# brodbeck-m/dolfinx_eqlb

Measured on AMD Instinct MI355X. Metric: equilibrated patches/s (fp64) on 1M-tri Poisson k=2; L2 flux-divergence residual, higher is better.
Workload: dtype f64; 1 GPU; Poisson 1000000 triangles per GPU (crossed unit square 500x500), P2 primal, FluxEqlbSE RT2, homogeneous Dirichlet, fp64; headline=True, patches_per_gpu=501001, cells_per_gpu=1000000, nrhs=1, weak_symmetry=False, partition=none, solver=shuffle, scatter=tiled, accumulate=True

## Files before the change

### dolfinx_eqlb_amd/csrc/eqlb_internal.h

```cpp
#pragma once

#include <hip/hip_runtime.h>

#include <cstdint>
#include <string>
#include <map>
#include <mutex>
#include <vector>

#include "../../include/eqlb.h"

namespace eqlb
{

constexpr uint32_t INFO_FM_SHIFT = 0, INFO_FP_SHIFT = 2, INFO_LN_SHIFT = 4;
constexpr uint32_t INFO_REV_M = 1u << 6, INFO_REV_P = 1u << 7;
constexpr uint32_t INFO_LOCAL_SHIFT = 8;

constexpr uint8_t PFLAG_INTERIOR = 1, PFLAG_BC0 = 2, PFLAG_BCN = 4;
constexpr uint8_t PFLAG_WS_SKIP = 8, PFLAG_WS_GROUP = 16;
constexpr uint8_t PFLAG_WS_LEVEL_SHIFT = 5;
constexpr int WS_MAX_LEVELS = 4;
constexpr uint32_t INFO_GROUPROW_SHIFT = 8;

// ... 73 lines not shown
#endif
__host__ __device__ constexpr bool tile_spec_full(int K, int P) { return P <= 8 && K >= 2; }
__host__ __device__ constexpr bool tile_spec_interior(int K, int P)
{
  return EQLB_TILE_INTERIOR && ((K == 2 && (P == 8 || P == 16)) || (EQLB_TILE_INTERIOR_K3 && K == 3 && P == 8));
}
__host__ __device__ __forceinline__ int tile_wb_all(int n, int P) { return (n * P + 63) >> 6; }
__host__ __device__ __forceinline__ int tile_wb_whole(int n, int P) { return (n * P) >> 6; }
template <int P>
__host__ __device__ __forceinline__ void tile_nfix_range(const TileDesc& td, int B, int j, int& c0, int& c1)
{
  constexpr int PER = 64 / P;
  const int first = (j == 0) ? td.nfull[B] : td.nval[B][j - 1];
  c0 = (first + PER - 1) / PER;
  c1 = (EQLB_STRESS_NFIX && P - 1 - j >= 3) ? td.nval[B][j] / PER : 0;
  if (c1 < c0)
    c1 = c0;
}

struct TileArgs
{
  const TileDesc* tiles;
  const int32_t* tile_cells;
  int32_t ntiles, tc;
  const int32_t* facet_owner;
  const int32_t* cell_dofs;
  int64_t ndofs;
  int32_t nfacets;
  int32_t tile_first;
  int32_t accumulate;
  const double* basis_C;
  const double* basis_R;
};

constexpr int MULTI_RHS_MAX = 8;
struct MultiRhs
{
  int32_t n, rhs0;
  const double* g[MULTI_RHS_MAX];
  const double* f[MULTI_RHS_MAX];
  double* x[MULTI_RHS_MAX];
};

struct BuildArgs
{
  int32_t nnodes, nfacets, nrhs;
  const int32_t *cell_nodes, *cell_facets, *facet_nodes, *facet_cells_off, *facet_cells;
  const int32_t *node_cells_off, *node_facets_off, *node_facets;
  const uint8_t* facet_perm;
  const int8_t* facet_type;
  const int64_t* node_slot;
  const int64_t* node_patch;
  int64_t npatch_total;
  int32_t* slot_cell;
  uint32_t* slot_info;
  uint8_t* pn;
  uint8_t* pflag;
  const int8_t* node_ws;
  const int32_t* node_group;
  const int8_t* node_wslevel;
  int64_t ninst;
  const int32_t* inst_node;
  const int32_t* inst_slot;
  const int32_t* inst_tile;
  const int32_t* cell_tile;
  const int32_t* cell_pos;
  int32_t tile_cells;
  int32_t stride;
  int32_t *ex_ncells, *ex_cells, *ex_fcts;
  int8_t *ex_fl, *ex_il, *ex_rev;
  int32_t large;
};

void launch_build_patches(const BuildArgs& a, hipStream_t stream);
void launch_cell_geometry(int32_t ncells, const double* x, const int32_t* cell_nodes,
                          double* cellJ, hipStream_t stream);
int launch_se_patch(int k, int deg, int P, int solver, int scatter, const SeArgs& a,
                    hipStream_t stream, int mode = 0);
int launch_se_patch_fused(int k, int deg, int scatter, const SeArgs& a, const FusedBins& fb,
                          hipStream_t stream);
int launch_se_patch_tiled(int k, int deg, int mode, const SeArgs& a, const TileArgs& t, hipStream_t stream);
int launch_se_patch_tiled_multi(int k, int deg, int mode, const SeArgs& a, const TileArgs& t, const MultiRhs& mr,
                                hipStream_t stream);
int launch_se_patch_lowdeg(int k, int deg, int P, int solver, int scatter, const SeArgs& a, hipStream_t stream,
                           int mode);
int launch_se_patch_fused_lowdeg(int k, int deg, int scatter, const SeArgs& a, const FusedBins& fb,
                                 hipStream_t stream);
int launch_se_patch_tiled_lowdeg(int k, int deg, int mode, const SeArgs& a, const TileArgs& t, hipStream_t stream);
int launch_se_patch_tiled_multi_lowdeg(int k, int deg, int mode, const SeArgs& a, const TileArgs& t,
                                       const MultiRhs& mr, hipStream_t stream);
int launch_ev_patch_fused_lowdeg(int k, int deg, const SeArgs& a, const FusedBins& fb, hipStream_t stream);
int launch_se_patch_k4_lowdeg(int deg, int P, int solver, int scatter, const SeArgs& a, hipStream_t stream,
                              int mode);
int fill_tables_k4_lowdeg(int deg, std::vector<double>& out);
void launch_tile_facet_owner(const DeviceMesh& m, int64_t n, const int32_t* tile_cells, int32_t* code,
                             hipStream_t stream);
int tile_cells_of(int k);
int tile_cells_ev_of(int k);
int tile_cells_max_of(int k);
int launch_se_patch_large(int k, int deg, int mode, const SeArgs& a, const int32_t* off, double* ws,
                          hipStream_t stream);
size_t large_patch_ws_doubles(int k, int64_t nslots, int64_t npatch);
int launch_se_weaksym_large(int k, const SeArgs& a, const int32_t* off, const int64_t* wsoff, double* ws,
                            hipStream_t stream);
size_t large_patch_weaksym_ws_doubles(int k, int64_t ncells_of_patch);
int launch_se_weaksym(int k, int P, bool no_flux_bcs, const SeArgs& a, hipStream_t stream);
int launch_se_weaksym_banded(int k, int P, const SeArgs& a, hipStream_t stream);
int launch_se_stress_tiled(const SeArgs& a, const TileArgs& t, const double* const* g, const double* const* f,
                           double* const* x, hipStream_t stream, bool mixed = false);
int stress_tile_cells();
int launch_ev_patch_fused(int k, int deg, const SeArgs& a, const FusedBins& fb, hipStream_t stream);
void launch_ev_boundary_to_broken(const DeviceMesh& m, int k, int nrhs, const int32_t* cell_dofs,
                                  int64_t ndofs, const double* bv_conf, double* bv_broken,
                                  const double* facet_maps, hipStream_t stream);
void launch_ev_reduce(const DeviceMesh& m, int k, int nrhs, const int32_t* cell_dofs, int64_t ndofs,
                      const double* slots, double* x, int accumulate, const double* basis_C, const double* basis_R,
                      hipStream_t stream);
int launch_reduce_slots(int nrt, int32_t ncells, int32_t nrhs, const double* slots, double* x, int accumulate,
                        hipStream_t stream);
int launch_reduce_slots_cells(int nrt, int32_t ncells, int64_t nlist, const int32_t* cells, const double* slots,
                              double* x, hipStream_t stream);
int projection_matrix_host(int degree, int nq, const double* pts, const double* wts,
                           std::vector<double>& Pm);
void launch_project_dg(int64_t ncells, int nd, int nq, int bs, const double* Pm, const double* qv,
                       double* out, hipStream_t stream);
void launch_korn(const DeviceMesh& m, const int64_t* node_slot, const int64_t* node_patch,
                 const int32_t* slot_cell, const uint32_t* slot_info, const uint8_t* pn,
                 const uint8_t* pflag, double* cks, double* korn, hipStream_t stream, int64_t l_npatch = 0,
                 const int32_t* l_nodes = nullptr, const int32_t* l_off = nullptr, const int32_t* l_slot_cell = nullptr,
                 const uint32_t* l_slot_info = nullptr, const uint8_t* l_pflag = nullptr);
int launch_estimate(const DeviceMesh& m, int k, int deg, int nrhs, const double* x_eq, const double* flux_dg,
                    const double* rhs_dg, double* div2, double* sig2, double* jump, double alpha,
                    double beta, hipStream_t stream);
int launch_boundary_residual(const DeviceMesh& m, int k, int deg, int nrhs, const double* x_eq,
                             const double* flux_dg, int32_t nlist, const int32_t* facets, const double* bvals,
                             double* out, hipStream_t stream);
int launch_estimate_stress(const DeviceMesh& m, const int32_t* node_cells, int k, const double* x0,
                           const double* x1, const double* korn, double pi_1, double* energy, double* wsym,
                           double* node_asym, hipStream_t stream);
int launch_oscillation(const DeviceMesh& m, int k, int deg, int nrhs, const double* x_eq, const double* flux_dg,
                       int nq, const double* qpoints, const double* qweights, const double* fvalues,
                       const double* korn, double* out, hipStream_t stream);
int launch_estimate_lowdeg(const DeviceMesh& m, int k, int deg, int nrhs, const double* x_eq, const double* flux_dg,
                           const double* rhs_dg, double* div2, double* sig2, double* jump, double alpha,
                           double beta, hipStream_t stream);
int launch_boundary_residual_lowdeg(const DeviceMesh& m, int k, int deg, int nrhs, const double* x_eq,
                                    const double* flux_dg, int32_t nlist, const int32_t* facets,
                                    const double* bvals, double* out, hipStream_t stream);
int launch_oscillation_lowdeg(const DeviceMesh& m, int k, int deg, int nrhs, const double* x_eq,
                              const double* flux_dg, int nq, const double* qpoints, const double* qweights,
                              const double* fvalues, const double* korn, double* out, hipStream_t stream);
int launch_estimate_k4_lowdeg(const DeviceMesh& m, int deg, int nrhs, const double* x_eq, const double* flux_dg,
                              const double* rhs_dg, double* div2, double* sig2, double* jump, double alpha,
                              double beta, hipStream_t stream);
int launch_boundary_residual_k4_lowdeg(const DeviceMesh& m, int deg, int nrhs, const double* x_eq,
                                       const double* flux_dg, int32_t nlist, const int32_t* facets,
                                       const double* bvals, double* out, hipStream_t stream);
int launch_oscillation_k4_lowdeg(const DeviceMesh& m, int deg, int nrhs, const double* x_eq, const double* flux_dg,
                                 int nq, const double* qpoints, const double* qweights, const double* fvalues,
                                 const double* korn, double* out, hipStream_t stream);
int set_error(int code, const char* fmt, ...);
void launch_halo_pack(int nrhs, int32_t nlist, int32_t nrt, int64_t ncells, const int64_t* cells, double* x,
                      double* buf, int clear, hipStream_t stream);
void launch_halo_unpack_add(int nrhs, int32_t nlist, int32_t nrt, int64_t ncells, const int64_t* cells,
                            double* x, const double* buf, hipStream_t stream);
void device_tiling_prepare();
// ... 115 lines not shown
```

### dolfinx_eqlb_amd/csrc/eqlb_se_kernels.hip

```cpp
#include "eqlb_device_common.h"
#include "eqlb_tables_gen.h"

#ifndef EQLB_PCR_SELECTS
#define EQLB_PCR_SELECTS 0
#endif

#ifndef EQLB_SE_TEMPLATES_ONLY
#define EQLB_SE_TEMPLATES_ONLY 0
#endif

namespace eqlb
{

#if !EQLB_SE_TEMPLATES_ONLY
size_t table_doubles(int k, int deg)
{
  const int nrt = nrt_of(k), nd = nd_of(deg), nq = nq_of(k);
  const int kb = k - 1, nadd = (k - 1) * (k - 2) / 2, ndiv = k * (k + 1) / 2 - 1;
  const int nh = 1 + 2 * kb + nadd, ncol = 2 * k + ndiv;
  const int hrow = nd * nq + ((nd * nq) & 1);
  const int nte = nh * (nh + 1) / 2;
  return (size_t)3 * nrt * nrt + (size_t)9 * nd * k + (size_t)3 * hrow + (size_t)6 * nd * nq
         + (size_t)NCOMBO * 3 * (nte + (nte & 1)) + (size_t)NCOMBO * 3 * nh * (ncol + (ncol & 1))
         + (size_t)9 * k * k + (size_t)3 * nrt * 2 + (size_t)NCOMBO * 2 * nh * 3
// ... 1841 lines not shown
{
  const int64_t e = (int64_t)blockIdx.x * blockDim.x + threadIdx.x;
  if (e >= n)
    return;
  const int32_t c = tile_cells[e / 3];
  const int lf = (int)(e % 3);
  int32_t v = -1;
  if (c >= 0)
  {
    const int32_t fct = cell_facets[(int64_t)c * 3 + lf];
    if (facet_cells[facet_cells_off[fct]] == c)
      v = 2 * fct + (facet_perm[(int64_t)c * 3 + lf] ? 1 : 0);
  }
  code[e] = v;
}

void launch_tile_facet_owner(const DeviceMesh& m, int64_t n, const int32_t* tile_cells, int32_t* code,
                             hipStream_t stream)
{
  if (n > 0)
    hipLaunchKernelGGL(k_tile_facet_owner, dim3((unsigned)((n + 255) / 256)), dim3(256), 0, stream, n,
                       tile_cells, m.cell_facets, m.facet_cells_off, m.facet_cells, m.facet_perm, code);
}
#endif

__device__ __forceinline__ int xcd_remap(int b, int n)
{
#if EQLB_XCD_REMAP
  const int q = n / 8, r = n % 8, x = b % 8;
  return ((x < r) ? x * (q + 1) : r * (q + 1) + (x - r) * q) + b / 8;
#else
  return b;
#endif
}

template <int K, int NPK>
__device__ __forceinline__ double packed_sum(const double* rows, int i)
{
  if (i >= 3 * K)
  {
    const int q = i - K;
    return (rows[q] + rows[NPK + q]) + rows[2 * NPK + q];
  }
  const int f = i / K, j = i - f * K;
  const int la = (f == 0) ? 1 : 0, lb = (f == 2) ? 1 : 2;
  return rows[la * NPK + (f - ((f > la) ? 1 : 0)) * K + j] + rows[lb * NPK + (f - ((f > lb) ? 1 : 0)) * K + j];
}

template <int K, int DEG, int MODE>
__device__ __forceinline__ void tile_stage(const SeArgs& a0, const TileArgs& ta, const int tile, double* lds)
{
  constexpr int TILE_THREADS = tile_threads_c(K);
  using Z = Sizes<K, DEG, 8>;
  constexpr int NRT = Z::NRT;
  const int TC = ta.tc;
  constexpr int NPK = NRT - K;
  constexpr bool HALFWQ = K == 3;
  constexpr int NTABL = HALFWQ ? Z::NTAB_HALF : Z::NTAB;
  constexpr int NTABM = NTABL + (MODE ? Z::NEV : 0);
  double* sSlots = lds + NTABM;
  if constexpr (HALFWQ)
  {
    constexpr int NHEAD = Z::NF + Z::NHT + Z::NDT + Z::NTET;
    constexpr int NCMB = Z::NCMB;
    for (int i = threadIdx.x; i < NHEAD; i += TILE_THREADS)
      lds[i] = a0.tables[Z::NS + i];
    for (int i = threadIdx.x; i < (NCOMBO / 2) * NCMB; i += TILE_THREADS)
      lds[NHEAD + (i / NCMB) * Z::NCMBH + (i % NCMB)] = a0.tables[Z::NS + NHEAD + (i / NCMB) * 2 * NCMB + (i % NCMB)];
    for (int i = threadIdx.x; i < Z::NHB; i += TILE_THREADS)
      lds[NHEAD + Z::NWQH + i] = a0.tables[Z::NS + NHEAD + Z::NWQT + i];
  }
  else
    for (int i = threadIdx.x; i < Z::NTAB; i += TILE_THREADS)
      lds[i] = a0.tables[Z::NS + i];
  if constexpr (MODE == 1)
    for (int i = threadIdx.x; i < Z::NEV; i += TILE_THREADS)
      lds[NTABL + i] = a0.tables[Z::OFF_HG + i];
  if (ta.tiles[tile].zero)
    for (int i = threadIdx.x; i < TC * 3 * NPK; i += TILE_THREADS)
      sSlots[i] = 0.0;
  __syncthreads();
}

template <int K, int DEG, int MODE>
__device__ __forceinline__ void tile_sweep_flush(const SeArgs& a0, const TileArgs& ta, const int tile, double* lds)
{
  constexpr int TILE_THREADS = tile_threads_c(K);
  using Z = Sizes<K, DEG, 8>;
  constexpr int NRT = Z::NRT;
  constexpr int TCMAX = tile_cells_max_c(K);
  const int TC = ta.tc;
  constexpr int NPK = NRT - K;
  constexpr bool HALFWQ = K == 3;
  constexpr int NTABL = HALFWQ ? Z::NTAB_HALF : Z::NTAB;
  constexpr int NTABM = NTABL + (MODE ? Z::NEV : 0);
  double* sSlots = lds + NTABM;
  const TileDesc& td = ta.tiles[tile];
#ifndef EQLB_TILE_SOLVER
#define EQLB_TILE_SOLVER 1
#endif
#ifndef EQLB_EXP_FULLONLY
#define EQLB_EXP_FULLONLY 0
#endif
  const int wave = threadIdx.x >> 6, lane = threadIdx.x & 63;
  constexpr int NW = TILE_THREADS / 64;
  int u = wave;
  SeArgs a = a0;
#define EQLB_TILE_BIN(B, PP)                                                                        \
  {                                                                                                 \
    const int np = td.npatch[B];                                                                    \
    const int nwb = tile_wb_all(np, PP);                                                            \
    a.npatch = np;                                                                                  \
    a.slot_offset = td.slot_start[B];                                                               \
    a.patch_offset = td.patch_start[B];                                                             \
     \
    constexpr bool SPEC = tile_spec_full(K, PP);                                                    \
    const int nwb_full = SPEC ? tile_wb_whole(td.nfull[B], PP) : 0;                                 \
     \
    constexpr bool SPECI = tile_spec_interior(K, PP);                                               \
    const int nwb_int = SPECI ? tile_wb_whole(td.nint[B], PP) : 0;                                  \
    for (; u < nwb; u += NW)                                                                        \
    {                                                                                               \
      if (u < nwb_full)                                                                             \
        se_patch_body<K, DEG, PP, EQLB_TILE_SOLVER, 2, 64, MODE, SPEC>(a, 0, lds, true, (int64_t)u * 64 + lane, sSlots); \
      else if (SPECI && u < nwb_int)                                                                \
        se_patch_body<K, DEG, PP, EQLB_TILE_SOLVER, 2, 64, MODE, false, SPECI>(a, 0, lds, true, (int64_t)u * 64 + lane, sSlots); \
      else if (!EQLB_EXP_FULLONLY)             \
        se_patch_body<K, DEG, PP, EQLB_TILE_SOLVER, 2, 64, MODE>(a, 0, lds, true, (int64_t)u * 64 + lane, sSlots); \
    }                                                                                               \
    u -= nwb;                                                                                       \
  }
#ifndef EQLB_EXP_NOBODY
  EQLB_TILE_BIN(0, 4)
  EQLB_TILE_BIN(1, 8)
  EQLB_TILE_BIN(2, 16)
  EQLB_TILE_BIN(3, 32)
  EQLB_TILE_BIN(4, 64)
#else
  (void)u;
  (void)lane;
  (void)td;
#endif
#undef EQLB_TILE_BIN
  const int32_t* cells = ta.tile_cells + (int64_t)tile * TC;
  const bool conforming = MODE == 1 && ta.facet_owner != nullptr;
  double* x = a0.out + (int64_t)a0.rhs_out * a0.ncells * NRT;
  constexpr int VW = (NRT % 2 == 0) ? 2 : 1;
  constexpr int NIT = (TCMAX * NRT / VW + TILE_THREADS - 1) / TILE_THREADS;
  double xv[NIT][VW];
  int64_t xi[NIT];
  if (!conforming)
  {
#pragma unroll
    for (int it = 0; it < NIT; ++it)
    {
      const int e = (it * TILE_THREADS + threadIdx.x) * VW;
      const int cl = e / NRT, i = e - cl * NRT;
      const int32_t cell = (e < TC * NRT) ? cells[cl] : -1;
      xi[it] = (cell >= 0) ? (int64_t)cell * NRT + i : -1;
    }
#pragma unroll
    for (int it = 0; it < NIT; ++it)
    {
#ifdef EQLB_EXP_NOXREAD
      xv[it][0] = xv[it][VW - 1] = 0.0;
      continue;
#endif
      if (!ta.accumulate)
      {
        xv[it][0] = xv[it][VW - 1] = 0.0;
        continue;
      }
      if constexpr (VW == 2)
      {
#if EQLB_FLUSH_NT
        xv[it][0] = (xi[it] >= 0) ? __builtin_nontemporal_load(x + xi[it]) : 0.0;
        xv[it][1] = (xi[it] >= 0) ? __builtin_nontemporal_load(x + xi[it] + 1) : 0.0;
#else
        const double2 t = (xi[it] >= 0) ? *reinterpret_cast<const double2*>(x + xi[it]) : make_double2(0.0, 0.0);
        xv[it][0] = t.x;
        xv[it][1] = t.y;
#endif
      }
      else
        xv[it][0] = (xi[it] >= 0) ? x[xi[it]] : 0.0;
    }
  }
  constexpr int NIC = K * K - K;
  constexpr int NFE = (TCMAX * 3 + TILE_THREADS - 1) / TILE_THREADS;
  constexpr int NIE = (NIC > 0) ? (TCMAX * NIC + TILE_THREADS - 1) / TILE_THREADS : 1;
  int32_t fcode[NFE];
  int64_t fdof[NFE];
  double fold[NFE][K];
  int64_t idof[NIE];
  double iold[NIE];
  const bool conf_plain = conforming && ta.basis_C == nullptr;
  if (conf_plain)
  {
    const double* xc0 = a0.out + (int64_t)a0.rhs_out * ta.ndofs;
    const int32_t* own0 = ta.facet_owner + (int64_t)tile * TC * 3;
#pragma unroll
    for (int it = 0; it < NFE; ++it)
    {
      const int e = it * TILE_THREADS + threadIdx.x;
      fcode[it] = (e < TC * 3) ? own0[e] : -1;
    }
#pragma unroll
    for (int it = 0; it < NFE; ++it)
    {
      const int e = it * TILE_THREADS + threadIdx.x;
      const int cl = e / 3, lf = e - 3 * cl;
      fdof[it] = -1;
      if (fcode[it] >= 0)
        fdof[it] = ta.cell_dofs ? (int64_t)cells[cl] * NRT + lf * K : (int64_t)(fcode[it] >> 1) * K;
#pragma unroll
      for (int j = 0; j < K; ++j)
      {
        fold[it][j] = 0.0;
        if (fcode[it] >= 0 && ta.accumulate)
          fold[it][j] = ta.cell_dofs ? xc0[ta.cell_dofs[fdof[it] + j]] : xc0[fdof[it] + j];
      }
    }
    if constexpr (NIC > 0)
    {
#pragma unroll
      for (int it = 0; it < NIE; ++it)
// ... 184 lines not shown
  using Z = Sizes<K, DEG, 8>;
  const size_t lds_bytes
      = sizeof(double) * ((size_t)(K == 3 ? Z::NTAB_HALF : Z::NTAB) + (MODE ? (size_t)Z::NEV : 0) + (size_t)t.tc * 3 * (Z::NRT - K));
  if (lds_bytes > 160 * 1024 || t.tc < 1 || t.tc > tile_cells_max_c(K) || mr.n < 1 || mr.n > MULTI_RHS_MAX)
    return EQLB_ERR_UNSUPPORTED;
  auto kern = k_se_patch_tiled_multi<K, DEG, MODE>;
  if (lds_bytes > 64 * 1024)
  {
    if (hipFuncSetAttribute(reinterpret_cast<const void*>(kern),
                            hipFuncAttributeMaxDynamicSharedMemorySize, (int)lds_bytes) != hipSuccess)
      return EQLB_ERR_DEVICE;
  }
  if (t.ntiles == 0)
    return 0;
  hipLaunchKernelGGL(kern, dim3((unsigned)t.ntiles * (unsigned)mr.n), dim3(tile_threads_c(K)), lds_bytes, stream, a, t, mr);
  return (hipGetLastError() == hipSuccess) ? 0 : EQLB_ERR_DEVICE;
}

#if !EQLB_SE_TEMPLATES_ONLY
int launch_se_patch_tiled_multi(int k, int deg, int mode, const SeArgs& a, const TileArgs& t, const MultiRhs& mr,
                                hipStream_t stream)
{
  if (deg != k - 1)
    return launch_se_patch_tiled_multi_lowdeg(k, deg, mode, a, t, mr, stream);
  if (mode == 1)
  {
    if (k == 1)
      return launch_tiled_multi_kd<1, 0, 1>(a, t, mr, stream);
    if (k == 2)
      return launch_tiled_multi_kd<2, 1, 1>(a, t, mr, stream);
    if (k == 3)
      return launch_tiled_multi_kd<3, 2, 1>(a, t, mr, stream);
    return EQLB_ERR_UNSUPPORTED;
  }
  if (k == 1 && deg == 0)
    return launch_tiled_multi_kd<1, 0, 0>(a, t, mr, stream);
  if (k == 2 && deg == 1)
    return launch_tiled_multi_kd<2, 1, 0>(a, t, mr, stream);
  if (k == 3 && deg == 2)
    return launch_tiled_multi_kd<3, 2, 0>(a, t, mr, stream);
  return EQLB_ERR_UNSUPPORTED;
}
#endif

template <int K, int DEG, int MODE>
static int launch_tiled_kd(const SeArgs& a, const TileArgs& t, hipStream_t stream)
{
  using Z = Sizes<K, DEG, 8>;
  const size_t lds_bytes
      = sizeof(double) * ((size_t)(K == 3 ? Z::NTAB_HALF : Z::NTAB) + (MODE ? (size_t)Z::NEV : 0) + (size_t)t.tc * 3 * (Z::NRT - K));
  if (lds_bytes > 160 * 1024 || t.tc < 1 || t.tc > tile_cells_max_c(K))
    return EQLB_ERR_UNSUPPORTED;
  auto kern = k_se_patch_tiled<K, DEG, MODE>;
  if (lds_bytes > 64 * 1024)
  {
    if (hipFuncSetAttribute(reinterpret_cast<const void*>(kern),
                            hipFuncAttributeMaxDynamicSharedMemorySize, (int)lds_bytes) != hipSuccess)
      return EQLB_ERR_DEVICE;
  }
  if (t.ntiles == 0)
    return 0;
  hipLaunchKernelGGL(kern, dim3((unsigned)t.ntiles), dim3(tile_threads_c(K)), lds_bytes, stream, a, t);
  return (hipGetLastError() == hipSuccess) ? 0 : EQLB_ERR_DEVICE;
}

#if !EQLB_SE_TEMPLATES_ONLY
int launch_se_patch_tiled(int k, int deg, int mode, const SeArgs& a, const TileArgs& t, hipStream_t stream)
{
  if (deg != k - 1)
    return launch_se_patch_tiled_lowdeg(k, deg, mode, a, t, stream);
  if (mode == 1)
  {
    if (k == 1)
      return launch_tiled_kd<1, 0, 1>(a, t, stream);
    if (k == 2)
      return launch_tiled_kd<2, 1, 1>(a, t, stream);
    if (k == 3)
      return launch_tiled_kd<3, 2, 1>(a, t, stream);
    return EQLB_ERR_UNSUPPORTED;
  }
  if (k == 1 && deg == 0)
    return launch_tiled_kd<1, 0, 0>(a, t, stream);
  if (k == 2 && deg == 1)
    return launch_tiled_kd<2, 1, 0>(a, t, stream);
  if (k == 3 && deg == 2)
    return launch_tiled_kd<3, 2, 0>(a, t, stream);
  return EQLB_ERR_UNSUPPORTED;
}

template <int NRT>
__global__ void __launch_bounds__(256)
k_reduce_slots(int64_t ntotal, const double* __restrict__ slots, double* __restrict__ x, int accumulate)
{
  const int64_t e = (int64_t)blockIdx.x * blockDim.x + threadIdx.x;
  if (e >= ntotal)
    return;
  const int64_t c = e / NRT;
  const int i = (int)(e - c * NRT);
  const double* s = slots + c * 3 * NRT + i;
  const double v = (s[0] + s[NRT]) + s[2 * NRT];
  x[e] = accumulate ? x[e] + v : v;
}

int launch_reduce_slots(int nrt, int32_t ncells, int32_t nrhs, const double* slots, double* x, int accumulate,
                        hipStream_t stream)
{
  const int64_t ntotal = (int64_t)nrhs * ncells * nrt;
  const int block = 256;
  const int64_t grid = (ntotal + block - 1) / block;
  if (nrt == 3)
    hipLaunchKernelGGL(k_reduce_slots<3>, dim3(grid), dim3(block), 0, stream, ntotal, slots, x, accumulate);
  else if (nrt == 8)
    hipLaunchKernelGGL(k_reduce_slots<8>, dim3(grid), dim3(block), 0, stream, ntotal, slots, x, accumulate);
  else if (nrt == 15)
    hipLaunchKernelGGL(k_reduce_slots<15>, dim3(grid), dim3(block), 0, stream, ntotal, slots, x, accumulate);
  else if (nrt == 24)
    hipLaunchKernelGGL(k_reduce_slots<24>, dim3(grid), dim3(block), 0, stream, ntotal, slots, x, accumulate);
  else
    return EQLB_ERR_UNSUPPORTED;
  return 0;
}

template <int NRT>
__global__ void __launch_bounds__(256)
k_reduce_slots_cells(int64_t ntotal, const int32_t* __restrict__ cells, const double* __restrict__ slots,
                     double* __restrict__ x)
{
  const int64_t e = (int64_t)blockIdx.x * blockDim.x + threadIdx.x;
  if (e >= ntotal)
    return;
  const int64_t c = cells[e / NRT];
  const int i = (int)(e % NRT);
  const double* s = slots + c * 3 * NRT + i;
  x[c * NRT + i] += (s[0] + s[NRT]) + s[2 * NRT];
}

int launch_reduce_slots_cells(int nrt, int32_t ncells, int64_t nlist, const int32_t* cells, const double* slots,
                              double* x, hipStream_t stream)
{
  (void)ncells;
  const int64_t ntotal = nlist * nrt;
  if (ntotal == 0)
    return 0;
  const int block = 256;
  const int64_t grid = (ntotal + block - 1) / block;
  if (nrt == 8)
    hipLaunchKernelGGL(k_reduce_slots_cells<8>, dim3(grid), dim3(block), 0, stream, ntotal, cells, slots, x);
  else if (nrt == 3)
    hipLaunchKernelGGL(k_reduce_slots_cells<3>, dim3(grid), dim3(block), 0, stream, ntotal, cells, slots, x);
  else if (nrt == 15)
    hipLaunchKernelGGL(k_reduce_slots_cells<15>, dim3(grid), dim3(block), 0, stream, ntotal, cells, slots, x);
  else if (nrt == 24)
    hipLaunchKernelGGL(k_reduce_slots_cells<24>, dim3(grid), dim3(block), 0, stream, ntotal, cells, slots, x);
  else
    return EQLB_ERR_UNSUPPORTED;
  return 0;
}
#endif

template <int K, int DEG, int P, int SOLVER, int SCATTER, int MODE = 0>
static int launch_t(const SeArgs& a, hipStream_t stream)
{
  using Z = Sizes<K, DEG, P>;
  constexpr int BLOCK = Z::block_of(SOLVER);
  const size_t lds_bytes = sizeof(double) * (size_t)Z::lds_doubles(BLOCK, SOLVER, MODE);
  if (lds_bytes > 160 * 1024)
    return EQLB_ERR_UNSUPPORTED;
// ... 159 lines not shown
```

Measured before the change: 6.289 billion patches/s.

## Add paired-lane DPP solver for full 8-cell patches in tiled k=2 kernel

Adds a new tiled kernel path for k=2, deg=1, single RHS that handles full 8-cell interior patches with 4 lanes per patch. Each lane processes two cells, and the patch chain is solved cooperatively through DPP cross-lane shuffles instead of one lane per patch doing the whole serial solve. This is meant to cut per-lane register pressure and serial chain latency. In exchange it adds a separate code path, compiler fences to control scheduling, and readfirstlane uniformization of tile bin descriptors.

```diff
diff --git a/dolfinx_eqlb_amd/csrc/eqlb_internal.h b/dolfinx_eqlb_amd/csrc/eqlb_internal.h
--- a/dolfinx_eqlb_amd/csrc/eqlb_internal.h
+++ b/dolfinx_eqlb_amd/csrc/eqlb_internal.h
@@ -179,6 +179,17 @@
 int launch_se_patch_tiled(int k, int deg, int mode, const SeArgs& a, const TileArgs& t, hipStream_t stream);
 int launch_se_patch_tiled_multi(int k, int deg, int mode, const SeArgs& a, const TileArgs& t, const MultiRhs& mr,
                                 hipStream_t stream);
+#ifndef EQLB_PAIR_LANES
+#define EQLB_PAIR_LANES 1
+#endif
+#ifndef EQLB_PAIR_OPAQUE
+#define EQLB_PAIR_OPAQUE 0
+#endif
+#ifndef EQLB_PAIR_WQ_SPLIT
+#define EQLB_PAIR_WQ_SPLIT 1
+#endif
+bool pair_lanes_built();
+int launch_se_patch_tiled_pair(const SeArgs& a, const TileArgs& t, hipStream_t stream);
 int launch_se_patch_lowdeg(int k, int deg, int P, int solver, int scatter, const SeArgs& a, hipStream_t stream,
                            int mode);
 int launch_se_patch_fused_lowdeg(int k, int deg, int scatter, const SeArgs& a, const FusedBins& fb,
diff --git a/dolfinx_eqlb_amd/csrc/eqlb_pair_chain.h b/dolfinx_eqlb_amd/csrc/eqlb_pair_chain.h
--- /dev/null
+++ b/dolfinx_eqlb_amd/csrc/eqlb_pair_chain.h
@@ -0,0 +1,183 @@
+#pragma once
+
+#ifndef EQLB_PC_FN
+#if defined(__HIPCC__)
+#define EQLB_PC_FN __device__ __forceinline__
+#else
+#define EQLB_PC_FN inline
+#endif
+#endif
+
+namespace eqlb_pair
+{
+
+template <class T, class X>
+EQLB_PC_FN void rev2(const T& x0, const T& x1, const T& rho, T& y0, T& y1)
+{
+  y0 = x0;
+  y1 = X::fma(rho, X::fma(X::cst(-2.0), x1, x0), x1);
+}
+
+template <class T, class X>
+EQLB_PC_FN void pair_phase_b(const T (&gm)[2][2], const T (&gp)[2][2], const T (&rho_m)[2], const T (&rho_p)[2],
+                             const T (&sr0)[2], T (&mu_m)[2][2], T (&mu_p0)[2])
+{
+  T j0[2], j1[2], t0_, t1_;
+  rev2<T, X>(gm[1][0], gm[1][1], rho_p[0], t0_, t1_);
+  j0[0] = gp[0][0] + t0_;
+  j0[1] = gp[0][1] + t1_;
+  const T gn0 = X::up(gm[0][0]), gn1 = X::up(gm[0][1]);
+  rev2<T, X>(gn0, gn1, rho_p[1], t0_, t1_);
+  j1[0] = gp[1][0] + t0_;
+  j1[1] = gp[1][1] + t1_;
+  const T a0 = sr0[0] + X::dn(j1[0]);
+  const T a1 = sr0[1] + j0[0];
+  T s = a0 + a1;
+  s = s + X::z0(X::dn(s));
+  s = s + X::z01(X::dn2(s));
+  const T e = X::z0(X::dn(s));
+  const T t0 = e + a0, t1 = t0 + a1;
+  mu_p0[0] = t0;
+  mu_p0[1] = t1;
+  T v0, v1;
+  rev2<T, X>(X::dn(t1 + j1[0]), X::dn(j1[1]), rho_m[0], v0, v1);
+  mu_m[0][0] = -v0;
+  mu_m[0][1] = -v1;
+  rev2<T, X>(t0 + j0[0], j0[1], rho_m[1], v0, v1);
+  mu_m[1][0] = -v0;
+  mu_m[1][1] = -v1;
+}
+
+template <class T, class X>
+EQLB_PC_FN void cell_phase_b(const T (&gm)[2], const T (&gp)[2], const T& rho_m, const T& rho_p, const T& sr0,
+                             T (&mu_m)[2], T& mu_p0)
+{
+  T jv[2], t0_, t1_;
+  rev2<T, X>(X::up(gm[0]), X::up(gm[1]), rho_p, t0_, t1_);
+  jv[0] = gp[0] + t0_;
+  jv[1] = gp[1] + t1_;
+  T t = sr0 + X::dn(jv[0]);
+  t = t + X::pre(t, 1);
+  t = t + X::pre(t, 2);
+  t = t + X::pre(t, 4);
+  mu_p0 = t;
+  T v0, v1;
+  rev2<T, X>(X::dn(t + jv[0]), X::dn(jv[1]), rho_m, v0, v1);
+  mu_m[0] = -v0;
+  mu_m[1] = -v1;
+}
+
+template <class T, class X>
+EQLB_PC_FN void pair_chain(const T (&te)[2][6], const T (&le)[2][3], T& d, T& xe, T& xo, T& xn, typename X::mask& ok)
+{
+  const T alpha = X::qsum(te[0][0] + te[1][0]), rd = X::qsum(le[0][0] + le[1][0]);
+  const T bt_e = te[0][1] + X::dn(te[1][3]), rr_e = le[0][1] + X::dn(le[1][2]), dg_e = te[0][2] + X::dn(te[1][5]);
+  const T bt_o = te[1][1] + te[0][3], rr_o = le[1][1] + le[0][2], dg_o = te[1][2] + te[0][5];
+  const T off_e = te[0][4], off_o = te[1][4];
+  const T z10 = X::b0(bt_e), z11 = X::b0(dg_e), rz1 = X::b0(rr_e);
+  const T be = X::one0(dg_e), re0 = X::z0(rr_e), re1 = X::z0(bt_e);
+  const T ce = X::z0(off_e);
+  const T co = X::z3(off_o);
+  const T c0 = X::only0(off_e) + X::only3(off_o);
+  ok = X::pos(be);
+  const T ibe = X::rcp(be);
+  const T ibe_up = X::up(ibe), re0_up = X::up(re0), re1_up = X::up(re1), co_dn = X::dn(co);
+  const T fe = ce * ibe, fh = co * ibe_up;
+  T b = X::fma(-fh, co, X::fma(-fe, ce, dg_o));
+  T r0 = X::fma(-fh, re0_up, X::fma(-fe, re0, rr_o));
+  T r1 = X::fma(-fh, re1_up, X::fma(-fe, re1, bt_o));
+  T r2 = c0;
+  T am = -fe * co_dn;
+  {
+    ok = X::both(ok, X::pos(b));
+    const T ib = X::rcp(b);
+    const T ib_lo = X::dn(ib), a_lo = X::dn(am), r0_lo = X::dn(r0), r1_lo = X::dn(r1), r2_lo = X::dn(r2);
+    const T ib_hi = X::up(ib), cp = X::up(am), r0_hi = X::up(r0), r1_hi = X::up(r1), r2_hi = X::up(r2);
+    const T al = am * ib_lo, ga = cp * ib_hi;
+    b = X::fma(-ga, cp, X::fma(-al, am, b));
+    r0 = X::fma(-ga, r0_hi, X::fma(-al, r0_lo, r0));
+    r1 = X::fma(-ga, r1_hi, X::fma(-al, r1_lo, r1));
+    r2 = X::fma(-ga, r2_hi, X::fma(-al, r2_lo, r2));
+    am = -al * a_lo;
+  }
+  {
+    ok = X::both(ok, X::pos(b));
+    const T ib = X::rcp(b);
+    const T ib2 = X::dn2(ib), cp = X::dn2(am), r0_2 = X::dn2(r0), r1_2 = X::dn2(r1), r2_2 = X::dn2(r2);
+    const T al = am * ib2, ga = cp * ib2;
+    b = X::fma(-ga, cp, X::fma(-al, am, b));
+    const T w = al + ga;
+    r0 = X::fma(-w, r0_2, r0);
+    r1 = X::fma(-w, r1_2, r1);
+    r2 = X::fma(-w, r2_2, r2);
+  }
+  ok = X::both(ok, X::pos(b));
+  const T ibf = X::rcp(b);
+  const T so0 = r0 * ibf, so1 = r1 * ibf, so2 = r2 * ibf;
+  const T se0 = ibe * X::fma(-ce, so0, X::fma(-co_dn, X::dn(so0), re0));
+  const T se1 = ibe * X::fma(-ce, so1, X::fma(-co_dn, X::dn(so1), re1));
+  const T se2 = -ibe * X::fma(ce, so2, co_dn * X::dn(so2));
+  const T tred0 = X::qsum(X::fma(re1, se0, bt_o * so0)), tred1 = X::qsum(c0 * so0);
+  const T s00 = X::qsum(X::fma(re1, se1, bt_o * so1)), s10 = X::qsum(c0 * so1), s11 = X::qsum(c0 * so2);
+  const T l00 = alpha - s00, l10 = z10 - s10;
+  const T i0 = X::rcp(l00);
+  const T m = l10 * i0;
+  const T d1 = X::fma(-m, l10, z11 - s11);
+  ok = X::both(ok, X::both(X::pos(l00), X::pos(d1)));
+  const T q0 = rd - tred0;
+  const T q1 = X::fma(-m, q0, rz1 - tred1);
+  const T zz1 = q1 * X::rcp(d1);
+  const T zz0 = X::fma(-l10, zz1, q0) * i0;
+  d = zz0;
+  xo = X::fma(-so2, zz1, X::fma(-so1, zz0, so0));
+  xe = X::sel0(zz1, X::fma(-se2, zz1, X::fma(-se1, zz0, se0)));
+  xn = X::up(xe);
+}
+
+template <class T, class X>
+EQLB_PC_FN void cell_chain(const T (&te)[6], const T (&le)[3], T& d, T& xm, T& xp, typename X::mask& ok)
+{
+  const T alpha = X::gsum(te[0]), rd = X::gsum(le[0]);
+  const T bt = te[1] + X::dn(te[3]), rr = le[1] + X::dn(le[2]), dg = te[2] + X::dn(te[5]), off = te[4];
+  const T z10 = X::b0(bt), z11 = X::b0(dg), rz1 = X::b0(rr), off0 = X::b0(off);
+  T b = X::one0(dg), r0 = X::z0(rr), r1 = X::z0(bt);
+  const T offc = X::z0(X::zlast(off));
+  T r2 = X::only1(off0) + X::onlylast(off);
+  const T B1 = r1, B2 = r2;
+  T am = X::shr(offc, 1);
+  ok = X::pos(b);
+  for (int S = 1; S < 8; S *= 2)
+  {
+    ok = X::both(ok, X::pos(b));
+    const T ib = X::rcp(b);
+    const T ib_lo = X::shr(ib, S), a_lo = X::shr(am, S), r0_lo = X::shr(r0, S), r1_lo = X::shr(r1, S),
+            r2_lo = X::shr(r2, S);
+    const T ib_hi = X::shl(ib, S), cp = X::shl(am, S), r0_hi = X::shl(r0, S), r1_hi = X::shl(r1, S),
+            r2_hi = X::shl(r2, S);
+    const T al = am * ib_lo, ga = cp * ib_hi;
+    b = X::fma(-ga, cp, X::fma(-al, am, b));
+    r0 = X::fma(-ga, r0_hi, X::fma(-al, r0_lo, r0));
+    r1 = X::fma(-ga, r1_hi, X::fma(-al, r1_lo, r1));
+    r2 = X::fma(-ga, r2_hi, X::fma(-al, r2_lo, r2));
+    am = -al * a_lo;
+  }
+  ok = X::both(ok, X::pos(b));
+  const T ibf = X::rcp(b);
+  const T s0 = r0 * ibf, s1 = r1 * ibf, s2 = r2 * ibf;
+  const T tred0 = X::gsum(B1 * s0), tred1 = X::gsum(B2 * s0);
+  const T s00 = X::gsum(B1 * s1), s10 = X::gsum(B2 * s1), s11 = X::gsum(B2 * s2);
+  const T l00 = alpha - s00, l10 = z10 - s10;
+  const T i0 = X::rcp(l00);
+  const T m = l10 * i0;
+  const T d1 = X::fma(-m, l10, z11 - s11);
+  ok = X::both(ok, X::both(X::pos(l00), X::pos(d1)));
+  const T q0 = rd - tred0;
+  const T q1 = X::fma(-m, q0, rz1 - tred1);
+  const T zz1 = q1 * X::rcp(d1);
+  const T zz0 = X::fma(-l10, zz1, q0) * i0;
+  d = zz0;
+  xm = X::sel0(zz1, X::fma(-s2, zz1, X::fma(-s1, zz0, s0)));
+  xp = X::up(xm);
+}
+
+}
diff --git a/dolfinx_eqlb_amd/csrc/eqlb_se_kernels.hip b/dolfinx_eqlb_amd/csrc/eqlb_se_kernels.hip
--- a/dolfinx_eqlb_amd/csrc/eqlb_se_kernels.hip
+++ b/dolfinx_eqlb_amd/csrc/eqlb_se_kernels.hip
@@ -1947,7 +1947,10 @@
   __syncthreads();
 }
 
-template <int K, int DEG, int MODE>
+template <int K, int DEG>
+__device__ void se_pair_body(const SeArgs& a, int64_t slot_base, int lane, double* lds, double* tile_slots);
+
+template <int K, int DEG, int MODE, bool PAIR = false>
 __device__ __forceinline__ void tile_sweep_flush(const SeArgs& a0, const TileArgs& ta, const int tile, double* lds)
 {
   constexpr int TILE_THREADS = tile_threads_c(K);
@@ -1970,30 +1973,46 @@
   const int wave = threadIdx.x >> 6, lane = threadIdx.x & 63;
   constexpr int NW = TILE_THREADS / 64;
   int u = wave;
+  if constexpr (PAIR)
+    u = __builtin_amdgcn_readfirstlane(u);
   SeArgs a = a0;
+#define EQLB_TILE_UNI(x) (PAIR ? __builtin_amdgcn_readfirstlane(x) : (x))
 #define EQLB_TILE_BIN(B, PP)                                                                        \
   {                                                                                                 \
-    const int np = td.npatch[B];                                                                    \
+    const int np = EQLB_TILE_UNI(td.npatch[B]);                                                     \
     const int nwb = tile_wb_all(np, PP);                                                            \
     a.npatch = np;                                                                                  \
-    a.slot_offset = td.slot_start[B];                                                               \
-    a.patch_offset = td.patch_start[B];                                                             \
+    a.slot_offset = EQLB_TILE_UNI(td.slot_start[B]);                                                \
+    a.patch_offset = EQLB_TILE_UNI(td.patch_start[B]);                                              \
      \
     constexpr bool SPEC = tile_spec_full(K, PP);                                                    \
-    const int nwb_full = SPEC ? tile_wb_whole(td.nfull[B], PP) : 0;                                 \
+    const int nfull_b = EQLB_TILE_UNI(td.nfull[B]);                                                 \
+    const int nwb_full = SPEC ? tile_wb_whole(nfull_b, PP) : 0;                                     \
      \
     constexpr bool SPECI = tile_spec_interior(K, PP);                                               \
-    const int nwb_int = SPECI ? tile_wb_whole(td.nint[B], PP) : 0;                                  \
-    for (; u < nwb; u += NW)                                                                        \
+    const int nwb_int = SPECI ? tile_wb_whole(EQLB_TILE_UNI(td.nint[B]), PP) : 0;                   \
+     \
+                                                \
+    constexpr bool PAIRB = PAIR && PP == 8 && K == 2 && MODE == 0;                                  \
+    const int npair = PAIRB ? (nfull_b >> 4) : 0;                                                   \
+    const int nun = nwb - npair;                                                                    \
+    for (; u < nun; u += NW)                                                                        \
     {                                                                                               \
-      if (u < nwb_full)                                                                             \
-        se_patch_body<K, DEG, PP, EQLB_TILE_SOLVER, 2, 64, MODE, SPEC>(a, 0, lds, true, (int64_t)u * 64 + lane, sSlots); \
-      else if (SPECI && u < nwb_int)                                                                \
-        se_patch_body<K, DEG, PP, EQLB_TILE_SOLVER, 2, 64, MODE, false, SPECI>(a, 0, lds, true, (int64_t)u * 64 + lane, sSlots); \
+      if constexpr (PAIRB)                                                                          \
+        if (u < npair)                                                                              \
+        {                                                                                           \
+          se_pair_body<K, DEG>(a, (int64_t)u * 128, lane, lds, sSlots);                             \
+          continue;                                                                                 \
+        }                                                                                           \
+      const int v = u + npair;                                                                      \
+      if (v < nwb_full)                                                                             \
+        se_patch_body<K, DEG, PP, EQLB_TILE_SOLVER, 2, 64, MODE, SPEC>(a, 0, lds, true, (int64_t)v * 64 + lane, sSlots); \
+      else if (SPECI && v < nwb_int)                                                                \
+        se_patch_body<K, DEG, PP, EQLB_TILE_SOLVER, 2, 64, MODE, false, SPECI>(a, 0, lds, true, (int64_t)v * 64 + lane, sSlots); \
       else if (!EQLB_EXP_FULLONLY)             \
-        se_patch_body<K, DEG, PP, EQLB_TILE_SOLVER, 2, 64, MODE>(a, 0, lds, true, (int64_t)u * 64 + lane, sSlots); \
+        se_patch_body<K, DEG, PP, EQLB_TILE_SOLVER, 2, 64, MODE>(a, 0, lds, true, (int64_t)v * 64 + lane, sSlots); \
     }                                                                                               \
-    u -= nwb;                                                                                       \
+    u -= nun;                                                                                       \
   }
 #ifndef EQLB_EXP_NOBODY
   EQLB_TILE_BIN(0, 4)
@@ -2007,6 +2026,7 @@
   (void)td;
 #endif
 #undef EQLB_TILE_BIN
+#undef EQLB_TILE_UNI
   const int32_t* cells = ta.tile_cells + (int64_t)tile * TC;
   const bool conforming = MODE == 1 && ta.facet_owner != nullptr;
   double* x = a0.out + (int64_t)a0.rhs_out * a0.ncells * NRT;
@@ -2357,7 +2377,8 @@
   if (k == 1 && deg == 0)
     return launch_tiled_kd<1, 0, 0>(a, t, stream);
   if (k == 2 && deg == 1)
-    return launch_tiled_kd<2, 1, 0>(a, t, stream);
+    return (pair_lanes_built() && a.nrhs == 1) ? launch_se_patch_tiled_pair(a, t, stream)
+                                               : launch_tiled_kd<2, 1, 0>(a, t, stream);
   if (k == 3 && deg == 2)
     return launch_tiled_kd<3, 2, 0>(a, t, stream);
   return EQLB_ERR_UNSUPPORTED;
diff --git a/dolfinx_eqlb_amd/csrc/eqlb_se_kernels_pair.hip b/dolfinx_eqlb_amd/csrc/eqlb_se_kernels_pair.hip
--- /dev/null
+++ b/dolfinx_eqlb_amd/csrc/eqlb_se_kernels_pair.hip
@@ -0,0 +1,365 @@
+#include "eqlb_internal.h"
+
+#if EQLB_PAIR_LANES
+#define EQLB_SE_TEMPLATES_ONLY 1
+#include "eqlb_se_kernels.hip"
+#include "eqlb_pair_chain.h"
+
+namespace eqlb
+{
+
+struct PairDpp
+{
+  using mask = bool;
+  static __device__ __forceinline__ int sub()
+  {
+    int t = threadIdx.x;
+#if EQLB_PAIR_OPAQUE
+    asm volatile("" : "+v"(t));
+#endif
+    return t & 3;
+  }
+  static __device__ __forceinline__ double cst(double c) { return c; }
+  static __device__ __forceinline__ double fma(double a, double b, double c) { return __builtin_fma(a, b, c); }
+  static __device__ __forceinline__ double rcp(double a) { return rcp_d(a); }
+  static __device__ __forceinline__ bool pos(double a) { return a > 0.0; }
+  static __device__ __forceinline__ bool both(bool a, bool b) { return a && b; }
+  static __device__ __forceinline__ double dn(double v) { return dpp_d<0x93>(v); }
+  static __device__ __forceinline__ double up(double v) { return dpp_d<0x39>(v); }
+  static __device__ __forceinline__ double dn2(double v) { return dpp_d<0x4E>(v); }
+  static __device__ __forceinline__ double b0(double v) { return dpp_d<0x00>(v); }
+  static __device__ __forceinline__ double qsum(double v)
+  {
+    v += dpp_d<0xB1>(v);
+    v += dpp_d<0x4E>(v);
+    return v;
+  }
+  static __device__ __forceinline__ double z0(double v) { return (sub() == 0) ? 0.0 : v; }
+  static __device__ __forceinline__ double z01(double v) { return (sub() <= 1) ? 0.0 : v; }
+  static __device__ __forceinline__ double z3(double v) { return (sub() == 3) ? 0.0 : v; }
+  static __device__ __forceinline__ double one0(double v) { return (sub() == 0) ? 1.0 : v; }
+  static __device__ __forceinline__ double only0(double v) { return (sub() == 0) ? v : 0.0; }
+  static __device__ __forceinline__ double only3(double v) { return (sub() == 3) ? v : 0.0; }
+  static __device__ __forceinline__ double sel0(double a, double b) { return (sub() == 0) ? a : b; }
+};
+
+__device__ __forceinline__ void pair_fence(double& v) { asm volatile("" : "+v"(v)); }
+__device__ __forceinline__ void pair_fence(uint32_t& v) { asm volatile("" : "+v"(v)); }
+__device__ __forceinline__ void pair_fence(int& idx, double& r) { asm volatile("" : "+v"(idx), "+v"(r)); }
+template <int N>
+__device__ __forceinline__ void pair_fence(double (&v)[N])
+{
+#pragma unroll
+  for (int i = 0; i < N; ++i)
+    pair_fence(v[i]);
+}
+
+constexpr uint32_t PAIR_NEG = 1u << 31;
+struct PairDesc
+{
+  int fm, fp, ln, ci;
+  uint32_t loc;
+  double rho_m, rho_p, pf_m, pf_p, sgn;
+  __device__ __forceinline__ PairDesc(const uint32_t info)
+  {
+    sgn = (info & PAIR_NEG) ? -1.0 : 1.0;
+    fm = (info >> INFO_FM_SHIFT) & 3;
+    fp = (info >> INFO_FP_SHIFT) & 3;
+    ln = (info >> INFO_LN_SHIFT) & 3;
+    const bool rev_m = (info & INFO_REV_M) != 0, rev_p = (info & INFO_REV_P) != 0;
+    ci = combo_index(fm, fp, rev_m);
+    rho_m = rev_m ? 1.0 : 0.0;
+    rho_p = rev_p ? 1.0 : 0.0;
+    loc = (info & ~PAIR_NEG) >> INFO_LOCAL_SHIFT;
+    pf_m = (fm == 1) ? sgn : -sgn;
+    pf_p = (fp == 1) ? sgn : -sgn;
+  }
+};
+
+template <int K, int DEG>
+__device__ __forceinline__ void se_pair_body(const SeArgs& a, const int64_t slot_base, const int lane, double* lds,
+                                             double* tile_slots)
+{
+  static_assert(K == 2 && DEG == 1, "the pair-lane instance is written for RT_2 with P1 data");
+  using Z = Sizes<2, 1, 8>;
+  using X = PairDpp;
+  constexpr int ND = Z::ND, NQ = Z::NQ, NH = Z::NH, NCOL = Z::NCOL, NTES = Z::NTES, NCOLS = Z::NCOLS;
+  constexpr int NPK = Z::NRT - K;
+  static_assert(ND == 3 && NQ == 3 && NH == 3 && NCOL == 6 && NTES == 6 && NCOLS == 6 && NPK == 6, "RT_2 / P1 sizes");
+  const double* sF = lds;
+  const double* sH = sF + Z::NF;
+  const double* sTE = sH + Z::NHT + Z::NDT;
+  const double* sWQ = sTE + Z::NTET;
+
+  int l2 = 2 * lane;
+  asm volatile("" : "+v"(l2));
+  const int64_t slot = a.slot_offset + slot_base + l2;
+  const int2 cells = *reinterpret_cast<const int2*>(a.slot_cell + slot);
+  const uint2 infos = *reinterpret_cast<const uint2*>(a.slot_info + slot);
+  uint32_t info[2] = {infos.x, infos.y};
+  double Jc[2][4], gx[2][ND], gy[2][ND], fdat[2][ND];
+#pragma unroll
+  for (int c = 0; c < 2; ++c)
+  {
+    const int32_t cell = c ? cells.y : cells.x;
+    const double2* Jp = reinterpret_cast<const double2*>(a.cellJ + 4 * (int64_t)cell);
+    const double2* gp_ = reinterpret_cast<const double2*>(a.flux_dg + ((int64_t)a.rhs_in * a.ncells + cell) * (ND * 2));
+    const double* fp_ = a.rhs_dg + ((int64_t)a.rhs_in * a.ncells + cell) * ND;
+    const double2 j0 = Jp[0], j1 = Jp[1];
+#pragma unroll
+    for (int i = 0; i < ND; ++i)
+    {
+      const double2 g2 = gp_[i];
+      gx[c][i] = g2.x;
+      gy[c][i] = g2.y;
+    }
+#pragma unroll
+    for (int i = 0; i < ND; ++i)
+      fdat[c][i] = fp_[i];
+    Jc[c][0] = j0.x;
+    Jc[c][1] = j0.y;
+    Jc[c][2] = j1.x;
+    Jc[c][3] = j1.y;
+  }
+
+  double gm[2][K], gpv[2][K], Rq[2][NQ], met[2][3];
+#pragma unroll
+  for (int c = 0; c < 2; ++c)
+  {
+    if (c == 1)
+    {
+      pair_fence(gm[0]);
+      pair_fence(gpv[0]);
+      pair_fence(Rq[0]);
+      pair_fence(met[0]);
+      pair_fence(Jc[1]);
+      pair_fence(gx[1]);
+      pair_fence(gy[1]);
+      pair_fence(fdat[1]);
+      pair_fence(info[1]);
+    }
+    const int fm = (info[c] >> INFO_FM_SHIFT) & 3, fp = (info[c] >> INFO_FP_SHIFT) & 3;
+    int ln = (info[c] >> INFO_LN_SHIFT) & 3;
+    double gnm[ND], gnp[ND], wv[ND], pf_m, pf_p;
+    {
+      const double J00 = Jc[c][0], J01 = Jc[c][1], J10 = Jc[c][2], J11 = Jc[c][3];
+      const double detJ = J00 * J11 - J01 * J10;
+      info[c] |= (detJ > 0.0) ? 0u : PAIR_NEG;
+      const double sg = (detJ > 0.0) ? 1.0 : -1.0;
+      pf_m = (fm == 1) ? sg : -sg;
+      pf_p = (fp == 1) ? sg : -sg;
+      const double ia = rcp_d(fabs(detJ));
+      met[c][0] = (J00 * J00 + J10 * J10) * ia;
+      met[c][1] = (J00 * J01 + J10 * J11) * ia;
+      met[c][2] = (J01 * J01 + J11 * J11) * ia;
+      const double a00 = J11, a01 = -J01, a10 = -J10, a11 = J00;
+      const double nmx = (fm == 2) ? 0.0 : -1.0, nmy = (fm == 0) ? -1.0 : ((fm == 1) ? 0.0 : 1.0);
+      const double npx = (fp == 2) ? 0.0 : -1.0, npy = (fp == 0) ? -1.0 : ((fp == 1) ? 0.0 : 1.0);
+      const double num0 = a00 * nmx + a10 * nmy, num1 = a01 * nmx + a11 * nmy;
+      const double nup0 = a00 * npx + a10 * npy, nup1 = a01 * npx + a11 * npy;
+      double dvg = 0.0;
+#pragma unroll
+      for (int i = 0; i < ND; ++i)
+      {
+        const double g2x = gx[c][i], g2y = gy[c][i];
+        gnm[i] = g2x * num0 + g2y * num1;
+        gnp[i] = g2x * nup0 + g2y * nup1;
+        const double gh0 = a00 * g2x + a01 * g2y;
+        const double gh1 = a10 * g2x + a11 * g2y;
+        wv[i] = detJ * fdat[c][i];
+        if (i == 0)
+          dvg = -(gh0 + gh1);
+        else if (i == 1)
+          dvg += gh0;
+        else
+          dvg += gh1;
+      }
+#pragma unroll
+      for (int i = 0; i < ND; ++i)
+        wv[i] -= dvg;
+    }
+#pragma unroll
+    for (int j = 0; j < K; ++j)
+      gm[c][j] = gpv[c][j] = 0.0;
+#pragma unroll
+    for (int q = 0; q < NQ; ++q)
+      Rq[c][q] = 0.0;
+    pair_fence(ln, wv[ND - 1]);
+    pair_fence(gnm);
+    pair_fence(gnp);
+    pair_fence(met[c]);
+    {
+      const double* tF_m = row16<true>(sF + (fm * 3 + ln) * ND * K);
+      const double* tF_p = row16<true>(sF + (fp * 3 + ln) * ND * K);
+#pragma unroll
+      for (int i = 0; i < ND; ++i)
+      {
+        double rm[K], rp[K];
+        ldrow16<K>(tF_m + i * K, rm);
+        ldrow16<K>(tF_p + i * K, rp);
+#pragma unroll
+        for (int j = 0; j < K; ++j)
+        {
+          gm[c][j] += rm[j] * gnm[i];
+          gpv[c][j] += rp[j] * gnp[i];
+        }
+      }
+#pragma unroll
+      for (int j = 0; j < K; ++j)
+      {
+        gm[c][j] *= pf_m;
+        gpv[c][j] *= pf_p;
+      }
+    }
+    pair_fence(gm[c]);
+    pair_fence(ln, gpv[c][K - 1]);
+    {
+      const double* tH = row16<true>(sH + ln * Z::HROW);
+      double rH[Z::HROW];
+      ldrow16<Z::HROW>(tH, rH);
+#pragma unroll
+      for (int i = 0; i < ND; ++i)
+#pragma unroll
+        for (int q = 0; q < NQ; ++q)
+          Rq[c][q] += wv[i] * rH[i * NQ + q];
+    }
+  }
+
+  double mu_m[2][K], mu_p0[2];
+  {
+    const double rho_m[2] = {(info[0] & INFO_REV_M) ? 1.0 : 0.0, (info[1] & INFO_REV_M) ? 1.0 : 0.0};
+    const double rho_p[2] = {(info[0] & INFO_REV_P) ? 1.0 : 0.0, (info[1] & INFO_REV_P) ? 1.0 : 0.0};
+    const double sr0[2] = {(info[0] & PAIR_NEG) ? -Rq[0][0] : Rq[0][0], (info[1] & PAIR_NEG) ? -Rq[1][0] : Rq[1][0]};
+    eqlb_pair::pair_phase_b<double, X>(gm, gpv, rho_m, rho_p, sr0, mu_m, mu_p0);
+  }
+
+  double te[2][NTES], le[2][NH];
+#pragma unroll
+  for (int c = 0; c < 2; ++c)
+  {
+    if (c == 1)
+    {
+      pair_fence(te[0]);
+      pair_fence(le[0]);
+      pair_fence(met[1]);
+      pair_fence(mu_m[1]);
+      pair_fence(mu_p0[1]);
+      pair_fence(Rq[1]);
+    }
+    pair_fence(info[c]);
+    const PairDesc p(info[c]);
+    const double g0 = met[c][0], g1 = met[c][1], g2 = met[c][2];
+    int ci = p.ci;
+    pair_fence(ci, mu_p0[c]);
+    const double* tep = row16<true>(sTE + ci * 3 * NTES);
+#pragma unroll
+    for (int e2 = 0; e2 < NTES / 2; ++e2)
+    {
+      const double2 t0 = reinterpret_cast<const double2*>(tep)[e2];
+      const double2 t1 = reinterpret_cast<const double2*>(tep + NTES)[e2];
+      const double2 t2 = reinterpret_cast<const double2*>(tep + 2 * NTES)[e2];
+      te[c][2 * e2] = g0 * t0.x + g1 * t1.x + g2 * t2.x;
+      te[c][2 * e2 + 1] = g0 * t0.y + g1 * t1.y + g2 * t2.y;
+    }
+    pair_fence(te[c]);
+    const double full[NCOL] = {mu_m[c][0], mu_m[c][1], mu_p0[c], 0.0, p.sgn * Rq[c][1], p.sgn * Rq[c][2]};
+#pragma unroll
+    for (int h = 0; h < NH; ++h)
+    {
+      double sx[3];
+#pragma unroll
+      for (int x = 0; x < 3; ++x)
+      {
+#if EQLB_PAIR_WQ_SPLIT
+        pair_fence(ci, (x > 0) ? sx[x - 1] : ((h == 0) ? te[c][NTES - 1] : le[c][h - 1]));
+#else
+        if (x == 0)
+          pair_fence(ci, (h == 0) ? te[c][NTES - 1] : le[c][h - 1]);
+#endif
+        const double* wq = row16<true>(sWQ + ci * 3 * NH * NCOLS + (x * NH + h) * NCOLS);
+        double s_ = 0.0;
+#pragma unroll
+        for (int c2 = 0; c2 < NCOLS / 2; ++c2)
+        {
+          const double2 w = reinterpret_cast<const double2*>(wq)[c2];
+          s_ = __builtin_fma(w.x, full[2 * c2], s_);
+          if (2 * c2 + 1 != K + 1)
+            s_ = __builtin_fma(w.y, full[2 * c2 + 1], s_);
+        }
+        sx[x] = s_;
+      }
+      le[c][h] = -(g0 * sx[0] + g1 * sx[1] + g2 * sx[2]);
+    }
+    if (p.loc != 0u)
+    {
+      double* o = tile_slots + ((int64_t)(p.loc - 1) * 3 + p.ln) * NPK;
+      o[2 * K] = Rq[c][1];
+      o[2 * K + 1] = Rq[c][2];
+    }
+  }
+
+  double d, xe, xo, xn;
+  bool posdef;
+  eqlb_pair::pair_chain<double, X>(te, le, d, xe, xo, xn, posdef);
+  if (!posdef)
+    atomicOr(a.status, 1);
+
+#pragma unroll
+  for (int c = 0; c < 2; ++c)
+  {
+    pair_fence(info[c]);
+    const PairDesc p(info[c]);
+    if (p.loc == 0u)
+      continue;
+    const double um = c ? xo : xe, up = c ? xn : xo;
+    double u0, u1;
+    eqlb_pair::rev2<double, X>(d, um, p.rho_m, u0, u1);
+    const double ym[K] = {mu_m[c][0] - u0, mu_m[c][1] - u1};
+    const double yp[K] = {mu_p0[c] + d, up};
+    double* o = tile_slots + ((int64_t)(p.loc - 1) * 3 + p.ln) * NPK;
+    const int pm = p.fm - ((p.fm > p.ln) ? 1 : 0), pp = p.fp - ((p.fp > p.ln) ? 1 : 0);
+#pragma unroll
+    for (int j = 0; j < K; ++j)
+    {
+      o[pm * K + j] = p.pf_m * ym[j];
+      o[pp * K + j] = p.pf_p * yp[j];
+    }
+  }
+}
+
+__global__ void __launch_bounds__(tile_threads_c(2), 4) k_se_patch_tiled_pair(const SeArgs a0, const TileArgs ta)
+{
+  extern __shared__ __align__(16) double lds[];
+  const int tile = ta.tile_first + xcd_remap(blockIdx.x, ta.ntiles);
+  tile_stage<2, 1, 0>(a0, ta, tile, lds);
+  tile_sweep_flush<2, 1, 0, true>(a0, ta, tile, lds);
+}
+
+bool pair_lanes_built() { return true; }
+
+int launch_se_patch_tiled_pair(const SeArgs& a, const TileArgs& t, hipStream_t stream)
+{
+  using Z = Sizes<2, 1, 8>;
+  const size_t lds_bytes = sizeof(double) * ((size_t)Z::NTAB + (size_t)t.tc * 3 * (Z::NRT - 2));
+  if (lds_bytes > 160 * 1024 || t.tc < 1 || t.tc > tile_cells_max_c(2))
+    return EQLB_ERR_UNSUPPORTED;
+  if (lds_bytes > 64 * 1024)
+  {
+    if (hipFuncSetAttribute(reinterpret_cast<const void*>(k_se_patch_tiled_pair),
+                            hipFuncAttributeMaxDynamicSharedMemorySize, (int)lds_bytes) != hipSuccess)
+      return EQLB_ERR_DEVICE;
+  }
+  if (t.ntiles == 0)
+    return 0;
+  hipLaunchKernelGGL(k_se_patch_tiled_pair, dim3((unsigned)t.ntiles), dim3(tile_threads_c(2)), lds_bytes, stream, a, t);
+  return (hipGetLastError() == hipSuccess) ? 0 : EQLB_ERR_DEVICE;
+}
+
+}
+#else
+namespace eqlb
+{
+bool pair_lanes_built() { return false; }
+int launch_se_patch_tiled_pair(const SeArgs&, const TileArgs&, hipStream_t) { return EQLB_ERR_UNSUPPORTED; }
+}
+#endif
```

Result: faster. 6.924 billion patches/s, median of 6 (+10.1%).
